# sumansamui/CMOOP_Audio_Processing

Measured on AMD Instinct MI355X. Metric: candidate-net evals/hour (pop=40, GSC-v2), higher is better.
Workload: dtype f32

## Files before the change

cmoop_audio_processing_amd/csrc/api.hip:

```cpp
#include "../../include/cmoop.h"
#include "net.h"

#include <cstring>
#include <mutex>
#include <vector>

using namespace cmoop;

static thread_local std::string g_err;
static thread_local std::string g_last_kernels;

template <class F>
static int guard(F&& f) {
    try {
        f();
        return 0;
    } catch (const std::exception& e) {
        g_err = e.what();
        return 1;
    } catch (...) {
        g_err = "unknown error";
        return 2;
    }
}
// ... 384 lines not shown
    return guard([&] {
        long long c = 0;
        h->net->read_train_metrics(loss_sum, &c, reset != 0);
        *correct = c;
    });
}
int cmoop_epoch_permutation(uint32_t seed, uint32_t epoch, int64_t n, int32_t* out_host) {
    return guard([&] { epoch_permutation(seed, epoch, n, out_host); });
}

int cmoop_epoch_permutation_device(uint32_t seed, uint32_t epoch, int64_t n, int32_t* out_dev) {
    return guard([&] {
        hipStream_t s = lib_stream();
        launch_epoch_permutation(seed, epoch, n, out_dev, s);
        CMOOP_HIP(hipStreamSynchronize(s));
    });
}


int cmoop_conv_fwd(const float* x, const float* w, const float* bias, float* y, int32_t B, int32_t H, int32_t W, int32_t Cin,
                   int32_t Cout, int32_t KS, int32_t stride, int32_t relu) {
    return guard([&] {
        g_last_kernels.clear();
        hipStream_t s = lib_stream();
        if (Cin == 1) {
            CMOOP_REQUIRE(stride == 1 && bias, "first-layer conv: stride 1 with bias");
            launch_conv1_fwd(x, nullptr, 0, w, bias, y, B, H, W, Cout, KS, relu, s);
        } else {
            GemmEpilogue e;
            e.bias = bias; e.relu = relu;
            const ConvGeom g = make_geom(B, H, W, Cin, Cout, KS, stride);
            const size_t skf = igemm_splitk_workspace(g);
            float* sk = nullptr;
            if (skf) CMOOP_HIP(hipMalloc(&sk, skf * 4));
            int flags = 0;
            const int code = launch_igemm_fwd(x, w, y, g, e, s, nullptr, sk, skf, nullptr, nullptr, 0, &flags);
            g_last_kernels = gemm_variant_name(0, code, flags);
            CMOOP_HIP(hipStreamSynchronize(s));
            if (sk) hipFree(sk);
        }
        CMOOP_HIP(hipStreamSynchronize(s));
    });
}

int cmoop_conv_bwd(const float* x, const float* w, const float* dy, float* dx, float* dw, float* db, int32_t B, int32_t H,
                   int32_t W, int32_t Cin, int32_t Cout, int32_t KS, int32_t stride, int32_t mask_relu) {
    return guard([&] {
        hipStream_t s = lib_stream();
        if (Cin == 1) {
            const int nb = conv1_wgrad_blocks(B, H, W);
            const int64_t per = (int64_t)Cout * (KS * KS + 1);
            float *P = nullptr, *tmp = nullptr;
            CMOOP_HIP(hipMalloc(&P, (size_t)nb * per * 4));
            CMOOP_HIP(hipMalloc(&tmp, (size_t)per * 4));
            launch_conv1_wgrad(x, nullptr, 0, dy, P, B, H, W, Cout, KS, s);
            launch_reduce_slices(P, tmp, nb, per, s);
            CMOOP_HIP(hipMemcpyAsync(dw, tmp, (size_t)Cout * KS * KS * 4, hipMemcpyDeviceToDevice, s));
            CMOOP_HIP(hipMemcpyAsync(db, tmp + (size_t)Cout * KS * KS, (size_t)Cout * 4, hipMemcpyDeviceToDevice, s));
            CMOOP_HIP(hipStreamSynchronize(s));
            hipFree(P); hipFree(tmp);
            return;
        }
        const ConvGeom g = make_geom(B, H, W, Cin, Cout, KS, stride);
        float *wg = nullptr, *red = nullptr, *wd = nullptr, *sk = nullptr;
        const size_t wg_floats = (size_t)wgrad_slices(g) * g.Cout * (g.K() + 1);
        CMOOP_HIP(hipMalloc(&wg, wg_floats * 4));
        CMOOP_HIP(hipMalloc(&red, ((size_t)1024 * 2 * Cout + 2 * Cout + 64) * 4));
        CMOOP_HIP(hipMalloc(&wd, (size_t)g.Cout * g.K() * 4));
        void* tab = nullptr;
        const int tab_rows = (KS * KS <= 32) ? rowtab_rows(g) : 0;
        if (tab_rows) {
            CMOOP_HIP(hipMalloc(&tab, (size_t)tab_rows * 8));
            launch_build_rowtab(g, tab, s);
        }
        g_last_kernels.clear();
        RecordingHook hook(&g_last_kernels);
        conv_backward_weights(x, dy, dw, db, g, wg, wg_floats, s, &hook, GEMM_DEFAULT, tab, tab_rows);
        if (dx) {
            int accumulate = 0;
            if (stride != 1) {
                CMOOP_HIP(hipMemsetAsync(dx, 0, (size_t)B * H * W * Cin * 4, s));
                accumulate = 1;
            }
            ConvGeom gd = g;
            gd.H = g.OH; gd.W = g.OW; gd.Cin = g.Cout; gd.Cout = g.Cin; gd.OH = g.H; gd.OW = g.W;
            const size_t skf = (stride == 1 && Cout >= 16 && (Cout & (Cout - 1)) == 0) ? igemm_splitk_workspace(gd) : 0;
            if (skf) CMOOP_HIP(hipMalloc(&sk, skf * 4));
            conv_backward_data(dy, w, dx, g, wd, mask_relu ? x : nullptr, 1.f, accumulate, s, &hook, sk, skf);
        }
        CMOOP_HIP(hipStreamSynchronize(s));
        hipFree(wg); hipFree(red); hipFree(wd);
        if (sk) hipFree(sk);
        if (tab) hipFree(tab);
    });
}

int cmoop_conv_fwd_trainer(const float* x, const float* w, const float* bias, float* y, int32_t B, int32_t H, int32_t W,
                           int32_t Cin, int32_t Cout, int32_t KS, int32_t stride, int32_t relu, double* col_sum,
                           double* col_sumsq, int32_t* stats_fused) {
    return guard([&] {
        g_last_kernels.clear();
        hipStream_t s = lib_stream();
        const ConvGeom g = make_geom(B, H, W, Cin, Cout, KS, stride);
        const int64_t M = g.M();
        GemmEpilogue e;
        e.bias = bias; e.relu = relu;
        float *sk = nullptr, *red = nullptr;
        void* tab = nullptr;
        const size_t skf = igemm_splitk_workspace(g);
        const bool want_stats = col_sum != nullptr && col_sumsq != nullptr;
        CMOOP_REQUIRE(!want_stats || Cout % 4 == 0, "statistics need Cout % 4 == 0");
        auto cleanup = [&] { hipStreamSynchronize(s); if (sk) hipFree(sk); if (red) hipFree(red); if (tab) hipFree(tab); };
        try {
            if (skf) CMOOP_HIP(hipMalloc(&sk, skf * 4));
            const int tab_rows = (KS * KS <= 32) ? rowtab_rows(g) : 0;
            if (tab_rows) {
                CMOOP_HIP(hipMalloc(&tab, (size_t)tab_rows * 8));
                launch_build_rowtab(g, tab, s);
            }
            size_t red_floats = 0;
            if (want_stats) {
                const size_t blocks = std::max<size_t>((size_t)colreduce_blocks(M, Cout), (size_t)cdiv64(M, 64));
                red_floats = blocks * 2 * Cout + 2 * Cout;
                CMOOP_HIP(hipMalloc(&red, red_floats * 4));
                e.stats = red;
            }
            int nb = 0, flags = 0;
            const int code = launch_igemm_fwd(x, w, y, g, e, s, nullptr, sk, skf, want_stats ? &nb : nullptr, tab, tab_rows, &flags);
            g_last_kernels = gemm_variant_name(0, code, flags);
            if (want_stats) {
                if (stats_fused) *stats_fused = nb > 0 ? 1 : 0;
                if (nb == 0) {
                    nb = colreduce_blocks(M, Cout);
                    launch_colstats(y, red, M, Cout, nb, s);
                }
                std::vector<float> hp((size_t)nb * 2 * Cout);
                CMOOP_HIP(hipMemcpyAsync(hp.data(), red, hp.size() * 4, hipMemcpyDeviceToHost, s));
                CMOOP_HIP(hipStreamSynchronize(s));
                for (int c = 0; c < Cout; ++c) { col_sum[c] = 0.0; col_sumsq[c] = 0.0; }
                for (int b = 0; b < nb; ++b)
                    for (int c = 0; c < Cout; ++c) {
                        col_sum[c] += (double)hp[((size_t)b * 2) * Cout + c];
                        col_sumsq[c] += (double)hp[((size_t)b * 2 + 1) * Cout + c];
                    }
            }
            CMOOP_HIP(hipStreamSynchronize(s));
        } catch (...) {
// ... 19 lines not shown
        try {
            RecordingHook hook(&g_last_kernels);
            const size_t NK = (size_t)g.Cout * g.K();
            const size_t wg_floats = (size_t)wgrad_slices(g) * g.Cout * (g.K() + 1);
            CMOOP_HIP(hipMalloc(&wg, wg_floats * 4));
            CMOOP_HIP(hipMalloc(&dwb, (NK + g.Cout) * 4));
            const int tab_rows = (KS * KS <= 32) ? rowtab_rows(g) : 0;
            if (tab_rows) {
                CMOOP_HIP(hipMalloc(&tab, (size_t)tab_rows * 8));
                launch_build_rowtab(g, tab, s);
            }
            conv_backward_weights(x, dy, dwb, dwb + NK, g, wg, wg_floats, s, &hook, GEMM_DEFAULT, tab, tab_rows);
            CMOOP_HIP(hipMemcpyAsync(dw, dwb, NK * 4, hipMemcpyDeviceToDevice, s));
            CMOOP_HIP(hipMemcpyAsync(db, dwb + NK, (size_t)g.Cout * 4, hipMemcpyDeviceToDevice, s));
            if (dx) {
                int accumulate = 0;
                if (stride != 1) {
                    CMOOP_HIP(hipMemsetAsync(dx, 0, (size_t)B * H * W * Cin * 4, s));
                    accumulate = 1;
                }
                const bool mfma_dgrad = ilog2_exact(Cout) >= 4;
                const ConvGeom gd = dgrad_geometry(g);
                int tab_d_rows = 0;
                size_t skf = 0;
                if (mfma_dgrad) {
                    CMOOP_HIP(hipMalloc(&wd, NK * 4));
                    launch_flip_transpose(w, wd, Cout, KS, KS, Cin, s);
                    if (KS * KS <= 32) {
                        tab_d_rows = rowtab_rows(gd);
                        CMOOP_HIP(hipMalloc(&tab_d, (size_t)tab_d_rows * 8));
                        launch_build_rowtab(gd, tab_d, s);
                    }
                    skf = igemm_splitk_workspace(gd);
                    if (skf) CMOOP_HIP(hipMalloc(&sk, skf * 4));
                }
                conv_backward_data(dy, w, dx, g, wd, mask_relu ? x : nullptr, 1.f, accumulate, s, &hook, sk, skf, GEMM_DEFAULT, mfma_dgrad,
                                   tab_d, tab_d_rows);
            }
            CMOOP_HIP(hipStreamSynchronize(s));
        } catch (...) {
            cleanup();
            throw;
        }
        cleanup();
    });
}

int cmoop_last_kernels(char* buf, int32_t cap) {
    return guard([&] {
        CMOOP_REQUIRE(buf && cap > 0, "last_kernels: no buffer");
        std::snprintf(buf, cap, "%s", g_last_kernels.c_str());
    });
}

int cmoop_conv_time(int32_t mode, const float* x, const float* w, const float* bias, float* y, int32_t B, int32_t H,
                    int32_t W, int32_t Cin, int32_t Cout, int32_t KS, int32_t iters, double* avg_ms) {
    return guard([&] {
        hipStream_t s = lib_stream();
        const ConvGeom g = make_geom(B, H, W, Cin, Cout, KS, 1);
        float *wd = nullptr, *wg = nullptr, *sk = nullptr;
        ConvGeom gd = g;
        GemmEpilogue e;
        const int S = wgrad_slices(g);
        if (mode == 0) e.bias = bias;
        if (mode == 1) {
            CMOOP_HIP(hipMalloc(&wd, (size_t)g.Cout * g.K() * 4));
            launch_flip_transpose(w, wd, Cout, KS, KS, Cin, s);
            gd.H = g.OH; gd.W = g.OW; gd.Cin = Cout; gd.Cout = Cin; gd.OH = g.H; gd.OW = g.W;
            gd.pad_t = KS - 1 - g.pad_t; gd.pad_l = KS - 1 - g.pad_l;
        }
        void* tab = nullptr;
        const int tab_rows = (KS * KS <= 32 && Cin >= 16) ? rowtab_rows(mode == 1 ? gd : g) : 0;
        if (mode == 2) CMOOP_HIP(hipMalloc(&wg, (size_t)S * g.Cout * g.K() * 4));
        if (tab_rows) {
            CMOOP_HIP(hipMalloc(&tab, (size_t)tab_rows * 8));
            launch_build_rowtab(mode == 1 ? gd : g, tab, s);
        }
        const size_t skf = mode == 0 ? igemm_splitk_workspace(g) : (mode == 1 ? igemm_splitk_workspace(gd) : 0);
        if (skf) CMOOP_HIP(hipMalloc(&sk, skf * 4));
        auto once = [&]() {
            if (mode == 0) launch_igemm_fwd(x, w, y, g, e, s, nullptr, sk, skf, nullptr, tab, tab_rows);
            else if (mode == 1) launch_igemm_fwd(y, wd, const_cast<float*>(x), gd, e, s, nullptr, sk, skf, nullptr, tab, tab_rows);
            else launch_igemm_wgrad(x, y, wg, g, S, s, nullptr, nullptr, 0, GEMM_DEFAULT, tab, tab_rows);
        };
        for (int i = 0; i < 3; ++i) once();
        hipEvent_t a, b;
        CMOOP_HIP(hipEventCreate(&a));
        CMOOP_HIP(hipEventCreate(&b));
        CMOOP_HIP(hipEventRecord(a, s));
        for (int i = 0; i < iters; ++i) once();
        CMOOP_HIP(hipEventRecord(b, s));
        CMOOP_HIP(hipEventSynchronize(b));
        float ms = 0.f;
        CMOOP_HIP(hipEventElapsedTime(&ms, a, b));
        hipEventDestroy(a); hipEventDestroy(b);
        if (wd) hipFree(wd);
        if (wg) hipFree(wg);
        if (sk) hipFree(sk);
        if (tab) hipFree(tab);
        *avg_ms = (double)ms / std::max(1, iters);
    });
}

int cmoop_dense_fwd(const float* x, const float* w, const float* bias, float* y, int32_t M, int32_t N, int32_t K, int32_t relu) {
    return guard([&] {
        hipStream_t s = lib_stream();
        launch_dense_fwd(x, w, bias, y, M, N, K, relu, 0, 0u, 0u, 1.f, GEMM_DEFAULT, s);
        CMOOP_HIP(hipStreamSynchronize(s));
    });
}
int cmoop_dense_bwd(const float* x, const float* w, const float* dy, float* dx, float* dw, float* db, int32_t M, int32_t N, int32_t K,
                    int32_t mask_relu) {
// ... 26 lines not shown
```

cmoop_audio_processing_amd/csrc/gemm.hip:

```cpp
#include "kernels.h"
#include <hip/hip_ext.h>
#include <cstdlib>
#include <mutex>
#include <string>
#include <type_traits>

namespace cmoop {

typedef float f32x4 __attribute__((ext_vector_type(4)));

typedef __bf16 bf16x8 __attribute__((ext_vector_type(8)));
typedef unsigned u32x4 __attribute__((ext_vector_type(4)));

typedef __bf16 bf16x2 __attribute__((ext_vector_type(2)));
typedef float f32x2 __attribute__((ext_vector_type(2)));

template <int NP>
__device__ __forceinline__ void split_pair(const float x, const float y, unsigned (&w)[NP]) {
    if constexpr (NP == 1) {
        w[0] = __builtin_bit_cast(unsigned, __builtin_convertvector((f32x2){x, y}, bf16x2));
    } else {
        const unsigned ux = __float_as_uint(x), uy = __float_as_uint(y);
        w[0] = __builtin_amdgcn_perm(uy, ux, 0x07060302u);
        const float rx = x - __uint_as_float(ux & 0xFFFF0000u), ry = y - __uint_as_float(uy & 0xFFFF0000u);
        const unsigned vx = __float_as_uint(rx), vy = __float_as_uint(ry);
        w[1] = __builtin_amdgcn_perm(vy, vx, 0x07060302u);
        const float sx = rx - __uint_as_float(vx & 0xFFFF0000u), sy = ry - __uint_as_float(vy & 0xFFFF0000u);
        w[2] = __builtin_amdgcn_perm(__float_as_uint(sy), __float_as_uint(sx), 0x07060302u);
    }
}

__device__ constexpr int X3_TA[6] = {2, 1, 0, 1, 0, 0};
__device__ constexpr int X3_TB[6] = {0, 1, 2, 0, 1, 0};

int gemm_mode_default() {
    static const int v = [] {
        const char* e = std::getenv("CMOOP_GEMM_MODE");
        if (!e) return (int)GEMM_FP32;
        const std::string m(e);
        return m == "bf16x3" ? (int)GEMM_BF16X3 : (m == "bf16" ? (int)GEMM_BF16 : (int)GEMM_FP32);
    }();
    return v;
}
static int resolve_mode(int mode) {
    const int m = mode >= 0 ? mode : gemm_mode_default();
    return (m == GEMM_BF16X3 || m == GEMM_BF16) ? m : GEMM_FP32;
}

struct GeomDev {
    int B, H, W, Cin, OH, OW, Cout, KH, KW, stride, pad_t, pad_l;
    int M, K, cshift, OHW;
    uint32_t ohw_magic, ohw_shift, ow_magic, ow_shift;
    int rcp_kw;
    const float* zeros;
};
struct EpiDev {
    int bal_L, bal_segmax;
    float* stats;
    const float* bias;
    const float* mask;
    float mask_scale;
    int relu, accumulate, out_stride, OHf, OWf, dropout;
    uint32_t drop_prefix, drop_thr;
    float drop_scale;
};

static double par_scale() {
    static const double v = [] {
        const char* e = std::getenv("CMOOP_PAR_SCALE");
        const double x = e ? std::atof(e) : 1.0;
        return x > 0.01 && x <= 4.0 ? x : 1.0;
    }();
    return v;
}

static void fastdiv_init(int d, uint32_t* magic, uint32_t* shift) {
    uint32_t s = 0;
    while ((1u << s) < (uint32_t)d) ++s;
    *shift = s;
    *magic = (uint32_t)((((uint64_t)1 << 32) * (((uint64_t)1 << s) - (uint64_t)d)) / (uint64_t)d + 1);
}
__device__ __forceinline__ int fastdiv(int n, uint32_t magic, uint32_t shift) {
    return (int)((__umulhi((uint32_t)n, magic) + (uint32_t)n) >> shift);
}

static const float* zero_page() {
    static thread_local const float* page[16] = {nullptr};
    int dev = 0;
    CMOOP_HIP(hipGetDevice(&dev));
    CMOOP_REQUIRE(dev >= 0 && dev < 16, "device index out of range");
// ... 569 lines not shown
                const int c = wcol + ct * 16 + lr;
                red[((wave / WN) * BN + c) * 2] = csum[ct];
                red[((wave / WN) * BN + c) * 2 + 1] = csq[ct];
            }
        }
        __syncthreads();
        if (t < BN && n0 + t < N) {
            float a = 0.f, b = 0.f;
#pragma unroll
            for (int w = 0; w < WM; ++w) { a += red[(w * BN + t) * 2]; b += red[(w * BN + t) * 2 + 1]; }
            e.stats[((size_t)mtile * 2) * N + n0 + t] = a;
            e.stats[((size_t)mtile * 2 + 1) * N + n0 + t] = b;
        }
    }
    }
}

struct HaloDev {
    int WP, rows_max, VH;
    uint32_t wp_magic, wp_shift, vh_magic, vh_shift;
};
__host__ __device__ constexpr int halo_nst(int bm) { return bm == 256 ? 11 : 9; }
static bool halo_geometry(const ConvGeom& cg, HaloDev* hd, size_t* lds_bytes);
static size_t halo_balanced_slab_floats(const ConvGeom& cg, int* L_out);

template <int KS, int BM, int BN, int WM, bool BAL = false>
__global__ __launch_bounds__(256, 2) void halo_fwd_kernel(const float* __restrict__ X, const float* __restrict__ Wt,
                                                          float* __restrict__ Y, GeomDev g, EpiDev e, HaloDev h,
                                                          float* __restrict__ slab) {
    constexpr int WN = 4 / WM, RT = BM / WM / 16, CT = BN / WN / 16, R = KS / 2, T = KS * KS;
    constexpr int PITCH = 24;
    constexpr int NST = halo_nst(BM);
    static_assert(RT >= 1 && CT >= 1, "tile too small for the wave layout");
    extern __shared__ __attribute__((aligned(16))) float halo[];

    const int t = threadIdx.x;
    const int ncc = g.Cin >> 4;
    const int upt = ncc * KS;
    int u = 0, uend = 1;
    if constexpr (BAL) {
        const int U = ((g.M + BM - 1) / BM) * ((g.Cout + BN - 1) / BN) * upt;
        u = blockIdx.x * e.bal_L;
        uend = min(U, u + e.bal_L);
    }
    while (u < uend) {
    int mtile, ntile, c_lo = 0, c_hi = upt;
    float* pslab = nullptr;
    if constexpr (BAL) {
        const int nt = (g.Cout + BN - 1) / BN;
        const int t0 = u / upt;
        c_lo = u - t0 * upt;
        c_hi = min(upt, c_lo + (uend - u));
        mtile = t0 / nt; ntile = t0 - mtile * nt;
        const int seg = c_lo == 0 ? 0 : (int)blockIdx.x - (t0 * upt) / e.bal_L;
        pslab = slab + ((size_t)t0 * e.bal_segmax + seg) * (BM * BN);
        u += c_hi - c_lo;
        __syncthreads();
    } else {
        u = uend;
        mtile = blockIdx.x;
        const int nwg = gridDim.x, xcd = mtile & 7, idx = mtile >> 3;
        const int qn = nwg >> 3, rn = nwg & 7;
        mtile = (xcd < rn ? xcd * (qn + 1) : rn * (qn + 1) + (xcd - rn) * qn) + idx;
        ntile = blockIdx.y;
    }
    const int m0 = mtile * BM, n0 = ntile * BN;
    const int wave = t >> 6, lane = t & 63, lr = lane & 15, q = lane >> 4;
    const int wrow = (wave / WN) * (BM / WM), wcol = (wave % WN) * (BN / WN);

    auto vrow = [&](int m, int& x) {
        const int b = fastdiv(m, g.ohw_magic, g.ohw_shift), r = m - b * g.OHW;
        const int y = fastdiv(r, g.ow_magic, g.ow_shift);
        x = r - y * g.OW;
        return b * h.VH + y;
    };
    int xdummy;
    const int vbase = vrow(m0, xdummy);
    const int vlast = vrow(min(m0 + BM, g.M) - 1, xdummy);
    const int items = (vlast - vbase + 1 + 2 * R) * h.WP * 4;

    const __amdgpu_buffer_rsrc_t xr = __builtin_amdgcn_make_buffer_rsrc(
        const_cast<float*>(X), 0, (int)((uint32_t)g.B * g.H * g.W << g.cshift) * 4, 0x00020000);
    const __amdgpu_buffer_rsrc_t wr = __builtin_amdgcn_make_buffer_rsrc(const_cast<float*>(Wt), 0, g.Cout * g.K * 4, 0x00020000);
    uint32_t s_voff[NST];
#pragma unroll
    for (int it = 0; it < NST; ++it) {
        const int i = t + 256 * it, pix = i >> 2, j = i & 3;
// ... 67 lines not shown
                    for (int rt = 0; rt < RT; ++rt)
                        an[rt] = *reinterpret_cast<const f32x4*>(a_ptr[rt] + ky * wp_f + (kx + 1) * PITCH);
                } else if (!last_unit) {
                    load_b(ncc2, nky * KS, bn);
                    if (!new_cc) {
#pragma unroll
                        for (int rt = 0; rt < RT; ++rt) an[rt] = *reinterpret_cast<const f32x4*>(a_ptr[rt] + nky * wp_f);
                    }
                }
                __builtin_amdgcn_s_setprio(1);
#pragma unroll
                for (int j = 0; j < 4; ++j)
#pragma unroll
                    for (int rt = 0; rt < RT; ++rt)
#pragma unroll
                        for (int ct = 0; ct < CT; ++ct)
                            acc[rt][ct] = __builtin_amdgcn_mfma_f32_16x16x4f32(ac[rt][j], bc[ct][j], acc[rt][ct], 0, 0, 0);
                __builtin_amdgcn_s_setprio(0);
#pragma unroll
                for (int ct = 0; ct < CT; ++ct) bc[ct] = bn[ct];
                if (kx + 1 < KS || (!last_unit && !new_cc)) {
#pragma unroll
                    for (int rt = 0; rt < RT; ++rt) ac[rt] = an[rt];
                } else if (!last_unit) {
                    __syncthreads();
                    stage_store();
                    __syncthreads();
#pragma unroll
                    for (int rt = 0; rt < RT; ++rt) ac[rt] = *reinterpret_cast<const f32x4*>(a_ptr[rt]);
                }
            }
            ky = nky; cc = ncc2;
        }
#pragma unroll
        for (int rt = 0; rt < RT; ++rt)
#pragma unroll
            for (int r = 0; r < 4; ++r)
#pragma unroll
                for (int ct = 0; ct < CT; ++ct)
                    pslab[(wrow + rt * 16 + q * 4 + r) * BN + wcol + ct * 16 + lr] = acc[rt][ct][r];
        continue;
    } else {
    f32x4 ac[RT], bc[CT];
    stage_load(0);
    load_b(0, 0, bc);
    stage_store();
    __syncthreads();
#pragma unroll
    for (int rt = 0; rt < RT; ++rt) ac[rt] = *reinterpret_cast<const f32x4*>(a_ptr[rt]);

    for (int cc = 0; cc < ncc; ++cc) {
        const bool more = cc + 1 < ncc;
#pragma unroll
        for (int tap = 0; tap < T; ++tap) {
            f32x4 an[RT], bn[CT];
#pragma unroll
            for (int ct = 0; ct < CT; ++ct) bn[ct] = bc[ct];
            if (tap + 1 < T) {
                load_b(cc, tap + 1, bn);
                const int ky = (tap + 1) / KS, kx = (tap + 1) % KS;
#pragma unroll
                for (int rt = 0; rt < RT; ++rt)
                    an[rt] = *reinterpret_cast<const f32x4*>(a_ptr[rt] + ky * wp_f + kx * PITCH);
            } else if (more) {
                load_b(cc + 1, 0, bn);
            }
            if (tap == T - 2 && more) stage_load(cc + 1);
            __builtin_amdgcn_s_setprio(1);
#pragma unroll
            for (int j = 0; j < 4; ++j)
#pragma unroll
                for (int rt = 0; rt < RT; ++rt)
#pragma unroll
                    for (int ct = 0; ct < CT; ++ct)
// ... 68 lines not shown
                    float v = (mk[r][ct] > 0.f) ? acc[rt][ct][r] * e.mask_scale : 0.f;
                    if (e.accumulate) v += old[r][ct];
                    __builtin_amdgcn_raw_buffer_store_b32(__float_as_uint(v), yrs, (int)(e_lane + ct * 64), soff, 0);
                }
        }
    } else {
#pragma unroll
    for (int rt = 0; rt < RT; ++rt) {
#pragma unroll
        for (int r = 0; r < 4; ++r) {
            const int row = m0 + wrow + rt * 16 + q * 4 + r;
            if (row >= g.M) continue;
            const size_t rbase = (size_t)row * N;
#pragma unroll
            for (int ct = 0; ct < CT; ++ct) {
                const int col = n0 + wcol + ct * 16 + lr;
                if (col >= N) continue;
                float v = acc[rt][ct][r] + bias_v[ct];
                if (e.relu) v = fmaxf(v, 0.f);
                const size_t off = rbase + col;
                if (e.dropout) {
                    uint32_t u24 = fmix32(e.drop_prefix ^ (uint32_t)((size_t)row * N + col)) >> 8;
                    v = (u24 >= e.drop_thr) ? v * e.drop_scale : 0.f;
                }
                if (e.mask) v = (e.mask[off] > 0.f) ? v * e.mask_scale : 0.f;
                if (e.accumulate) v += Y[off];
                Y[off] = v;
                csum[ct] += v;
                csq[ct] += v * v;
            }
        }
    }
    }
    if (e.stats) {
        __syncthreads();
        float* red = halo;
#pragma unroll
        for (int ct = 0; ct < CT; ++ct) {
            csum[ct] += __shfl_xor(csum[ct], 16, 64);
            csq[ct] += __shfl_xor(csq[ct], 16, 64);
            csum[ct] += __shfl_xor(csum[ct], 32, 64);
            csq[ct] += __shfl_xor(csq[ct], 32, 64);
            if (q == 0) {
                const int c = wcol + ct * 16 + lr;
                red[((wave / WN) * BN + c) * 2] = csum[ct];
                red[((wave / WN) * BN + c) * 2 + 1] = csq[ct];
            }
        }
        __syncthreads();
        if (t < BN && n0 + t < N) {
            float a = 0.f, b = 0.f;
#pragma unroll
            for (int w = 0; w < WM; ++w) { a += red[(w * BN + t) * 2]; b += red[(w * BN + t) * 2 + 1]; }
            e.stats[((size_t)mtile * 2) * N + n0 + t] = a;
            e.stats[((size_t)mtile * 2 + 1) * N + n0 + t] = b;
        }
    }
    }
}

struct BalDev { int bm, bn, nt, chunks, L, segmax; };

template <int VEC>
__global__ __launch_bounds__(256) void splitk_combine_kernel(const float* __restrict__ P, float* __restrict__ Y, GeomDev g,
                                                             EpiDev e, int splits, BalDev bal) {
    const int N = g.Cout;
    const size_t total = (size_t)g.M * N;
// ... 136 lines not shown
    if (balanced_on) {
        int W = 0;
        const size_t need = balanced_slab_floats(M, N, K, bk, bn_big, &W);
        if (need > 0 && need <= ws_floats) { *bm = 128; *bn = bn_big; *balanced_wgs = W; return; }
    }
    if (nchunks >= (M <= 512 ? 4 : 16) && ws_floats > 0) {
        const int min_chunks = M <= 512 ? 2 : 8;
        int sp = (int)std::min<long>(cdiv((int)(1024 * par_scale()), (int)blocks), nchunks / min_chunks);
        sp = std::min(sp, 32);
        if (sp > 1) sp = fill_waves(blocks, sp, std::max(32, (int)(512 * par_scale())));
        while (sp > 1 && (size_t)sp * M * N > ws_floats) --sp;
        if (sp > 1) {
            const int cps = cdiv(nchunks, sp);
            sp = cdiv(nchunks, cps);
            *bm = 128; *bn = bn_big; *splits = sp;
            return;
        }
    }
    blocks = (long)cdiv(M, 128) * cdiv(N, bn_small);
    if (blocks >= fill) { *bm = 128; *bn = bn_small; return; }
    *bm = 64; *bn = bn_small;
}

size_t igemm_splitk_workspace(const ConvGeom& g) {
    const int M = g.M(), N = g.Cout;
    const int bn_big = N > 64 ? 128 : (N <= 16 ? 16 : (N <= 32 ? 32 : 64));
    const long blocks = (long)cdiv(M, 128) * cdiv(N, bn_big);
    if (blocks >= 384) return 0;
    const int sp = std::min(32, cdiv(1024, (int)blocks));
    return std::max(std::max((size_t)sp * M * N, balanced_slab_floats(M, N, g.K(), g.Cin % 32 == 0 ? 32 : 16, bn_big, nullptr)),
                    halo_balanced_slab_floats(g, nullptr));
}

static size_t halo_balanced_slab_floats(const ConvGeom& cg, int* L_out) {
    static const bool on = [] { const char* v = std::getenv("CMOOP_HALO_BAL"); return !(v && v[0] == '0'); }();
    if (!on || cg.Cout % 64 != 0 || !halo_geometry(cg, nullptr, nullptr)) return 0;
    const long tiles = (long)cdiv(cg.M(), 128) * (cg.Cout / 64);
    const int upt = (cg.Cin / 16) * cg.KH;
    const long units = tiles * upt;
    if (tiles >= 1024 || units < 512l * 2 * cg.KH) return 0;
    const int L = (int)((units + 511) / 512);
    if (L_out) *L_out = L;
    return (size_t)tiles * (cdiv(upt, L) + 1) * 128 * 64;
}

struct FwdChoice {
    int mode, bm, bn, splits, balanced_wgs, flags;
    bool bk32_tile, use_dma, stats, halo;
    int ks, halo_L;
    int code() const { return mode * 100000000 + bm * 100000 + bn * 100 + (halo ? ks + (halo_L > 0 ? 50 : 0) : (bk32_tile ? 32 : 16)); }
};

static inline int halo_bm(int cout) { return cout >= 64 ? 128 : 256; }
static bool halo_geometry(const ConvGeom& cg, HaloDev* hd, size_t* lds_bytes) {
    const int ks = cg.KH, R = ks / 2;
    if (cg.KH != cg.KW || (ks != 3 && ks != 5) || cg.stride != 1 || cg.OH != cg.H || cg.OW != cg.W) return false;
    if (cg.pad_t != R || cg.pad_l != R || cg.Cin % 16 != 0) return false;
    if (cg.Cout % 64 != 0 && cg.Cout != 32 && cg.Cout != 16) return false;
    const int bm = halo_bm(cg.Cout);
    const int wp = (cg.W + ks - 1 + 7) / 8 * 8;
    const int span = (bm - 2 + cg.W) / cg.W + 1 + ((bm - 1) / (cg.H * cg.W) + 1) * R;
    const int rows = span + 2 * R;
    if (rows * wp * 4 > halo_nst(bm) * 256) return false;
    const size_t lds = (size_t)rows * wp * 24 * sizeof(float);
    if (lds > 64 * 1024) return false;
    if (hd) {
        hd->WP = wp; hd->rows_max = rows; hd->VH = cg.H + R;
        fastdiv_init(wp, &hd->wp_magic, &hd->wp_shift);
        fastdiv_init(cg.H + R, &hd->vh_magic, &hd->vh_shift);
    }
    if (lds_bytes) *lds_bytes = lds;
    return true;
}
// ... 41 lines not shown
        }
    }
    c.flags = (c.splits > 1 ? GEMM_FLAG_SPLITK : 0) | (c.stats ? GEMM_FLAG_STATS : 0) | (c.balanced_wgs ? GEMM_FLAG_BALANCED : 0) |
              ((!c.halo && have_rowtab && (cg.Cin % bk) == 0 && cg.KH * cg.KW <= 32) ? GEMM_FLAG_ROWTAB : 0);
    return c;
}

int igemm_fwd_plan(const ConvGeom& g, const GemmEpilogue& ep, size_t ws_floats, bool want_stats, bool have_rowtab, int* flags_out) {
    igemm_check_range(g);
    CMOOP_REQUIRE(ilog2_exact(g.Cin) >= 4, "implicit GEMM needs C_in a power of two >= 16");
    const FwdChoice c = choose_fwd(g, ep, ws_floats, want_stats, have_rowtab);
    if (flags_out) *flags_out = c.flags;
    return c.code();
}

int launch_igemm_fwd(const float* X, const float* Wt, float* Y, const ConvGeom& cg, const GemmEpilogue& ep,
                     hipStream_t s, const GemmTiming* tm, float* splitk_ws, size_t splitk_ws_floats, int* stats_blocks,
                     const void* rowtab_v, int tab_rows, int* flags_out) {
    if (stats_blocks) *stats_blocks = 0;
    if (flags_out) *flags_out = 0;
    const uint2* rowtab = static_cast<const uint2*>(rowtab_v);
    GeomDev g = to_dev(cg);
    if (g.M == 0) return 0;
    EpiDev e;
    e.bias = ep.bias; e.mask = ep.mask; e.mask_scale = ep.mask_scale; e.relu = ep.relu;
    e.accumulate = ep.accumulate; e.out_stride = ep.out_stride; e.OHf = ep.OHf; e.OWf = ep.OWf;
    e.dropout = ep.dropout; e.drop_prefix = ep.drop_prefix; e.drop_thr = ep.drop_thr; e.drop_scale = ep.drop_scale;
    if (e.out_stride > 1)
        CMOOP_REQUIRE((int64_t)g.B * e.OHf * e.OWf * g.Cout < (1ll << 29), "scattered output too large");
    const FwdChoice ch = choose_fwd(cg, ep, splitk_ws ? splitk_ws_floats : 0, ep.stats != nullptr && stats_blocks != nullptr, rowtab != nullptr);
    const int mode = ch.mode == GEMM_FP32_DMA ? (int)GEMM_FP32 : ch.mode;
    const int bm = ch.bm, bn = ch.bn, splits = ch.splits, balanced_wgs = ch.balanced_wgs;
    const bool bk32_tile = ch.bk32_tile, use_dma = ch.use_dma;
    e.bal_L = 0; e.bal_segmax = 0;
    e.stats = ch.stats ? ep.stats : nullptr;
    if (e.stats) *stats_blocks = cdiv(g.M, bm);
    if (flags_out) *flags_out = ch.flags;
    if (ch.halo) {
        HaloDev hd;
        size_t lds = 0;
        CMOOP_REQUIRE(halo_geometry(cg, &hd, &lds), "halo kernel chosen for a geometry it does not accept");
        dim3 grid(cdiv(g.M, bm), cdiv(g.Cout, bn));
        BalDev bal{bm, bn, cdiv(g.Cout, bn), (cg.Cin / 16) * cg.KH, ch.halo_L, 0};
        if (ch.halo_L > 0) {
            bal.segmax = cdiv(bal.chunks, bal.L) + 1;
            e.bal_L = bal.L; e.bal_segmax = bal.segmax;
            const long units = (long)grid.x * grid.y * bal.chunks;
            grid = dim3((unsigned)((units + bal.L - 1) / bal.L), 1, 1);
            lds = std::max(lds, (size_t)55 * 1024);
        }
        {
            static const int occ_env = [] { const char* v = std::getenv("CMOOP_HALO_OCC"); return v ? std::atoi(v) : 0; }();
            const long wgs = (long)grid.x * grid.y;
            auto fill = [&](long slots) { return (double)wgs / (double)(((wgs + slots - 1) / slots) * slots); };
            const bool two = occ_env == 2 || (occ_env != 3 && lds <= 53 * 1024 && wgs <= 1536 && fill(512) > fill(768) + 0.05);
            if (two) lds = std::max(lds, (size_t)55 * 1024);
        }
#define CMOOP_HALO_LAUNCH(KS_, BM_, BN_, WM_, BAL_)                                                                                        \
        do {                                                                                                                 \
            if (tm && tm->start && tm->ext) {                                                                                \
                hipExtLaunchKernelGGL((halo_fwd_kernel<KS_, BM_, BN_, WM_, BAL_>), grid, dim3(256), lds, s, tm->start, tm->stop, 0, X, Wt, Y, g, e, hd, splitk_ws); \
            } else {                                                                                                         \
                if (tm && tm->start) CMOOP_HIP(hipEventRecord(tm->start, s));                                                \
                hipLaunchKernelGGL((halo_fwd_kernel<KS_, BM_, BN_, WM_, BAL_>), grid, dim3(256), lds, s, X, Wt, Y, g, e, hd, splitk_ws);    \
                if (tm && tm->start) CMOOP_HIP(hipEventRecord(tm->stop, s));                                                 \
            }                                                                                                                \
        } while (0)
#define CMOOP_HALO_KS(KS_)                                                                     \
        do {                                                                                   \
            if (ch.halo_L > 0) CMOOP_HALO_LAUNCH(KS_, 128, 64, 2, true);                       \
            else if (bn == 64) CMOOP_HALO_LAUNCH(KS_, 128, 64, 2, false);                      \
            else if (bn == 32) CMOOP_HALO_LAUNCH(KS_, 256, 32, 4, false);                      \
            else CMOOP_HALO_LAUNCH(KS_, 256, 16, 4, false);                                    \
        } while (0)
        if (cg.KH == 5) CMOOP_HALO_KS(5); else CMOOP_HALO_KS(3);
#undef CMOOP_HALO_KS
#undef CMOOP_HALO_LAUNCH
        CMOOP_HIP(hipGetLastError());
        if (ch.halo_L > 0) {
            const size_t total = (size_t)g.M * g.Cout;
            const unsigned gridc = (unsigned)std::min<size_t>((total / 4 + 255) / 256, 4096);
            hipLaunchKernelGGL(splitk_combine_kernel<4>, dim3(gridc), dim3(256), 0, s, splitk_ws, Y, g, e, 2, bal);
            CMOOP_HIP(hipGetLastError());
        }
        return ch.code();
    }
#define CMOOP_FWD(BM_, BN_, WM_)                                                              \
    do {                                                                                      \
        if (mode == GEMM_BF16X3) launch_fwd_t<BM_, BN_, 32, WM_, GEMM_BF16X3>(X, Wt, Y, g, e, s, tm, splitk_ws, splits, balanced_wgs, rowtab, tab_rows);   \
        else if (mode == GEMM_BF16) launch_fwd_t<BM_, BN_, 32, WM_, GEMM_BF16>(X, Wt, Y, g, e, s, tm, splitk_ws, splits, balanced_wgs, rowtab, tab_rows);  \
        else if (use_dma && BM_ == 128 && BN_ == 32) launch_fwd_t<BM_, 32, 32, WM_, GEMM_FP32_DMA>(X, Wt, Y, g, e, s, tm, splitk_ws, splits, balanced_wgs, rowtab, tab_rows);   \
        else if (bk32_tile) launch_fwd_t<BM_, BN_, 32, WM_>(X, Wt, Y, g, e, s, tm, splitk_ws, splits, balanced_wgs, rowtab, tab_rows);   \
        else launch_fwd_t<BM_, BN_, 16, WM_>(X, Wt, Y, g, e, s, tm, splitk_ws, splits, 0, rowtab, tab_rows);        \
    } while (0)
    if (bm == 128) {
        if (bn == 128) CMOOP_FWD(128, 128, 2);
        else if (bn == 64) CMOOP_FWD(128, 64, 4);
        else if (bn == 32) CMOOP_FWD(128, 32, 4);
        else CMOOP_FWD(128, 16, 4);
    } else {
        if (bn == 64) CMOOP_FWD(64, 64, 2);
        else if (bn == 32) CMOOP_FWD(64, 32, 4);
        else CMOOP_FWD(64, 16, 4);
    }
#undef CMOOP_FWD
    return ch.code();
}

__global__ __launch_bounds__(256) void build_rowtab_kernel(GeomDev g, uint2* __restrict__ tab, int rows_padded) {
    const int m = blockIdx.x * 256 + threadIdx.x;
    if (m >= rows_padded) return;
    if (m >= g.M) { tab[m] = make_uint2(0u, 0xFFFFFFFFu); return; }
// ... 826 lines not shown
```

cmoop_audio_processing_amd/csrc/kernels.h:

```cpp
#pragma once
#include "common.h"
#include <string>

namespace cmoop {

struct ConvGeom {
    int B, H, W, Cin;
    int OH, OW, Cout;
    int KH, KW, stride;
    int pad_t, pad_l;
    int M() const { return B * OH * OW; }
    int K() const { return KH * KW * Cin; }
};

enum GemmMode { GEMM_DEFAULT = -1, GEMM_FP32 = 0, GEMM_FP32_DMA = 1 , GEMM_BF16X3 = 2, GEMM_BF16 = 3,
                GEMM_FP32_HALO = 4  };
int gemm_mode_default();

struct GemmEpilogue {
    int mode = GEMM_DEFAULT;
    const float* bias = nullptr;
    int relu = 0;
    const float* mask = nullptr;
    float mask_scale = 1.f;
    int accumulate = 0;
    int out_stride = 1;
    int OHf = 0, OWf = 0;
    int dropout = 0;
    uint32_t drop_prefix = 0, drop_thr = 0;
    float drop_scale = 1.f;
    float* stats = nullptr;
};

struct GemmTiming {
    hipEvent_t start = nullptr, stop = nullptr;
    bool ext = true;
};
enum GemmFlags { GEMM_FLAG_SPLITK = 1, GEMM_FLAG_STATS = 2, GEMM_FLAG_ROWTAB = 4, GEMM_FLAG_BALANCED = 8, GEMM_FLAG_SLABS = 16 };
int launch_igemm_fwd(const float* X, const float* Wt, float* Y, const ConvGeom& g,
                     const GemmEpilogue& e, hipStream_t s, const GemmTiming* tm = nullptr,
                     float* splitk_ws = nullptr, size_t splitk_ws_floats = 0, int* stats_blocks = nullptr,
                     const void* rowtab = nullptr, int tab_rows = 0, int* flags_out = nullptr);
size_t igemm_splitk_workspace(const ConvGeom& g);
int igemm_fwd_plan(const ConvGeom& g, const GemmEpilogue& e, size_t ws_floats, bool want_stats, bool have_rowtab, int* flags_out);
int igemm_wgrad_plan(const ConvGeom& g, int S, int mode, bool have_rowtab, int* flags_out);
void halo_rows_bound_and_need(const ConvGeom& g, int* bound, int* need, int* items_cap);
void igemm_check_range(const ConvGeom& g);
std::string gemm_kernel_name(int cls, int code);

int wgrad_slices(const ConvGeom& g);
int launch_igemm_wgrad(const float* X, const float* dY, float* P, const ConvGeom& g, int S, hipStream_t s,
                       const GemmTiming* tm = nullptr, float* Pbias = nullptr, size_t slab_stride = 0,
                       int mode = GEMM_DEFAULT, const void* rowtab = nullptr, int tab_rows = 0, int* flags_out = nullptr);
int rowtab_rows(const ConvGeom& g);
void launch_build_rowtab(const ConvGeom& g, void* tab, hipStream_t s);
void launch_reduce_slices(const float* P, float* out, int S, int64_t n, hipStream_t s, int64_t stride = 0);
void launch_flip_transpose(const float* W, float* Wd, int Cout, int KH, int KW, int Cin, hipStream_t s);
struct FlipEntry { int64_t w_off, wd_off; int Cout, KH, KW, Cin; };
void launch_flip_transpose_all(const float* params, float* wd_all, const FlipEntry* table_dev, int layers, int64_t max_elems,
                               hipStream_t s);

struct StepState {
    long long row0;
    unsigned step;
    unsigned iter;
};
void launch_step_advance(StepState* st, int batch, hipStream_t s);
void launch_glorot_init(float* w, int64_t n, uint32_t prefix, float scale, hipStream_t s);
void launch_fill(float* w, float v, int64_t n, hipStream_t s);

void launch_dense_fwd(const float* X, const float* W, const float* bias, float* Y, int M, int N, int K, int relu,
                      int dropout, uint32_t drop_prefix, uint32_t drop_thr, float drop_scale, int mode, hipStream_t s,
                      const StepState* st = nullptr, uint32_t drop_seed = 0, uint32_t drop_stream = 0);
void launch_dense_dgrad(const float* dY, const float* W, float* dX, int M, int N, int K, const float* mask, float mask_scale,
                        int mode, hipStream_t s);
void launch_dense_wgrad(const float* X, const float* dY, float* dW, float* dB, int M, int N, int K, int mode, hipStream_t s);
// ... 80 lines not shown
```

cmoop_audio_processing_amd/csrc/net.hip:

```cpp
#include "net.h"

#include <algorithm>
#include <chrono>
#include <cmath>
#include <cstdlib>
#include <cstring>
#include <functional>
#include <map>
#include <numeric>
#include <thread>

namespace cmoop {

static const int FC_LADDER[5][4] = {{0, 0, 0, 0}, {64, 0, 0, 0}, {128, 64, 0, 0}, {256, 128, 64, 0}, {512, 256, 128, 64}};

void validate_gene(const int32_t g[6]) {
    const bool ok = (g[0] == 16 || g[0] == 32 || g[0] == 64) && (g[1] == 3 || g[1] == 5) && (g[2] == 0 || g[2] == 1) &&
                    (g[3] >= 1 && g[3] <= 3) && (g[4] >= 1 && g[4] <= 4) && (g[5] == 0 || g[5] == 1);
    CMOOP_REQUIRE(ok, "gene outside the search space (filters{16,32,64}, kernel{3,5}, bn{0,1}, res{1..3}, fc{1..4}, dropout{0,1})");
}

int64_t param_count(const int32_t g[6], int variant, int classes) {
    validate_gene(g);
    const int64_t f = g[0], kk = (int64_t)g[1] * g[1], bn = g[2], R = g[3], fc = g[4];
// ... 335 lines not shown
            const int64_t M = g.M();
            if (op.Cout % 4 == 0)
                red_ws_floats_ = std::max(red_ws_floats_, (size_t)colreduce_blocks(M, op.Cout) * 2 * op.Cout + 2 * op.Cout);
        }
        if (op.kind == OP_CONV1) {
            const size_t per = (size_t)op.Cout * (op.KS * op.KS + 1);
            for (int b = 1; b <= cfg_.batch; ++b) op.slab_floats = std::max(op.slab_floats, per * conv1_wgrad_blocks(b, T_, F_));
            op.slab_off = (int64_t)wgrad_ws_floats_;
            wgrad_ws_floats_ += (op.slab_floats + 3) / 4 * 4;
            red_ws_floats_ = std::max(red_ws_floats_, (size_t)colreduce_blocks((int64_t)Bmax_ * T_ * F_, op.Cout) * 2 * op.Cout + 2 * op.Cout);
        }
        if (op.kind == OP_BN) {
            const int64_t M = (int64_t)Bmax_ * acts_[op.in].H * acts_[op.in].W;
            const size_t blocks = std::max<size_t>((size_t)colreduce_blocks(M, op.Cout), (size_t)cdiv64(M, 64));
            red_ws_floats_ = std::max(red_ws_floats_, blocks * 2 * op.Cout + 2 * op.Cout);
        }
    }
    wgrad_ws_ = dalloc(wgrad_ws_floats_);
    wd_ws_ = dalloc(wd_ws_floats_);
    {
        std::vector<FlipEntry> tab;
        for (const auto& op : ops_)
            if (op.kind == OP_CONV && op.wd_off >= 0) {
                tab.push_back(FlipEntry{op.w_off, op.wd_off, op.Cout, op.KS, op.KS, op.Cin});
                flip_max_elems_ = std::max<int64_t>(flip_max_elems_, (int64_t)op.Cout * op.KS * op.KS * op.Cin);
            }
        flip_layers_ = (int)tab.size();
        if (flip_layers_) {
            flip_table_ = reinterpret_cast<FlipEntry*>(dalloc(tab.size() * sizeof(FlipEntry) / sizeof(float) + 4));
            CMOOP_HIP(hipMemcpyAsync(flip_table_, tab.data(), tab.size() * sizeof(FlipEntry), hipMemcpyHostToDevice, stream_));
            CMOOP_HIP(hipStreamSynchronize(stream_));
        }
    }
    splitk_ws_ = splitk_ws_floats_ ? dalloc(splitk_ws_floats_) : nullptr;
    red_ws_ = dalloc(red_ws_floats_ + 64);
    acc_train_ = reinterpret_cast<double*>(dalloc(8));
    acc_eval_ = acc_train_ + 2;
    CMOOP_HIP(hipMemsetAsync(acc_train_, 0, 32, stream_));
    if (cfg_.profile_every > 0) {
        ev_pool_.resize(1024);
        const char* pm = std::getenv("CMOOP_PROFILE_PAIRS");
        const bool ext = !(pm && pm[0] == '1');
        static std::atomic<bool> said{false};
        if (!said.exchange(true)) std::fprintf(stderr, "[cmoop] GEMM launch timing: %s\n", ext ? "hipExtLaunchKernelGGL events" : "hipEventRecord pairs");
        for (auto& e : ev_pool_) {
            CMOOP_HIP(hipEventCreate(&e.t.start));
            CMOOP_HIP(hipEventCreate(&e.t.stop));
            e.t.ext = ext;
        }
    }
}

ConvGeom Net::geom_of(const Op& op, int B) const {
    const Act& ia = acts_[op.in];
    ConvGeom g;
    g.B = B; g.H = ia.H; g.W = ia.W; g.Cin = op.Cin;
    g.OH = (ia.H + op.stride - 1) / op.stride; g.OW = (ia.W + op.stride - 1) / op.stride; g.Cout = op.Cout;
    g.KH = g.KW = op.KS; g.stride = op.stride;
    const int th = std::max((g.OH - 1) * op.stride + op.KS - ia.H, 0);
    const int tw = std::max((g.OW - 1) * op.stride + op.KS - ia.W, 0);
    g.pad_t = th / 2; g.pad_l = tw / 2;
    return g;
}

void Net::get_params(float* host) {
    CMOOP_HIP(hipMemcpyAsync(host, params_, n_params_ * 4, hipMemcpyDeviceToHost, stream_));
    CMOOP_HIP(hipStreamSynchronize(stream_));
// ... 684 lines not shown
```

Measured before the change: 441.0.

## Fuse balanced halo split-K reduction into GEMM via per-tile atomic fix-up

Replaces the separate split-K combine kernel for the balanced halo GEMM with an in-kernel fix-up. Each segment stores its partial tile to the slab and bumps a per-tile atomic counter, and the last-arriving workgroup sums all partials and runs the normal epilogue. This removes one kernel launch and a full slab read/write pass over the output. In exchange it needs counter storage appended to the split-K workspace, a zeroing memset at allocation, and correct memory ordering. Fused stats are disabled on this path.

Result: no change. 443.8, median of 6 (+0.6%).

```diff
diff --git a/cmoop_audio_processing_amd/csrc/api.hip b/cmoop_audio_processing_amd/csrc/api.hip
--- a/cmoop_audio_processing_amd/csrc/api.hip
+++ b/cmoop_audio_processing_amd/csrc/api.hip
@@ -440,7 +440,10 @@
             const ConvGeom g = make_geom(B, H, W, Cin, Cout, KS, stride);
             const size_t skf = igemm_splitk_workspace(g);
             float* sk = nullptr;
-            if (skf) CMOOP_HIP(hipMalloc(&sk, skf * 4));
+            if (skf) {
+                CMOOP_HIP(hipMalloc(&sk, igemm_splitk_alloc_floats(skf) * 4));
+                igemm_splitk_zero_counters(sk, skf, s);
+            }
             int flags = 0;
             const int code = launch_igemm_fwd(x, w, y, g, e, s, nullptr, sk, skf, nullptr, nullptr, 0, &flags);
             g_last_kernels = gemm_variant_name(0, code, flags);
@@ -493,7 +496,10 @@
             ConvGeom gd = g;
             gd.H = g.OH; gd.W = g.OW; gd.Cin = g.Cout; gd.Cout = g.Cin; gd.OH = g.H; gd.OW = g.W;
             const size_t skf = (stride == 1 && Cout >= 16 && (Cout & (Cout - 1)) == 0) ? igemm_splitk_workspace(gd) : 0;
-            if (skf) CMOOP_HIP(hipMalloc(&sk, skf * 4));
+            if (skf) {
+                CMOOP_HIP(hipMalloc(&sk, igemm_splitk_alloc_floats(skf) * 4));
+                igemm_splitk_zero_counters(sk, skf, s);
+            }
             conv_backward_data(dy, w, dx, g, wd, mask_relu ? x : nullptr, 1.f, accumulate, s, &hook, sk, skf);
         }
         CMOOP_HIP(hipStreamSynchronize(s));
@@ -520,7 +526,10 @@
         CMOOP_REQUIRE(!want_stats || Cout % 4 == 0, "statistics need Cout % 4 == 0");
         auto cleanup = [&] { hipStreamSynchronize(s); if (sk) hipFree(sk); if (red) hipFree(red); if (tab) hipFree(tab); };
         try {
-            if (skf) CMOOP_HIP(hipMalloc(&sk, skf * 4));
+            if (skf) {
+                CMOOP_HIP(hipMalloc(&sk, igemm_splitk_alloc_floats(skf) * 4));
+                igemm_splitk_zero_counters(sk, skf, s);
+            }
             const int tab_rows = (KS * KS <= 32) ? rowtab_rows(g) : 0;
             if (tab_rows) {
                 CMOOP_HIP(hipMalloc(&tab, (size_t)tab_rows * 8));
@@ -606,7 +615,10 @@
                         launch_build_rowtab(gd, tab_d, s);
                     }
                     skf = igemm_splitk_workspace(gd);
-                    if (skf) CMOOP_HIP(hipMalloc(&sk, skf * 4));
+                    if (skf) {
+                        CMOOP_HIP(hipMalloc(&sk, igemm_splitk_alloc_floats(skf) * 4));
+                        igemm_splitk_zero_counters(sk, skf, s);
+                    }
                 }
                 conv_backward_data(dy, w, dx, g, wd, mask_relu ? x : nullptr, 1.f, accumulate, s, &hook, sk, skf, GEMM_DEFAULT, mfma_dgrad,
                                    tab_d, tab_d_rows);
@@ -651,7 +663,10 @@
             launch_build_rowtab(mode == 1 ? gd : g, tab, s);
         }
         const size_t skf = mode == 0 ? igemm_splitk_workspace(g) : (mode == 1 ? igemm_splitk_workspace(gd) : 0);
-        if (skf) CMOOP_HIP(hipMalloc(&sk, skf * 4));
+        if (skf) {
+            CMOOP_HIP(hipMalloc(&sk, igemm_splitk_alloc_floats(skf) * 4));
+            igemm_splitk_zero_counters(sk, skf, s);
+        }
         auto once = [&]() {
             if (mode == 0) launch_igemm_fwd(x, w, y, g, e, s, nullptr, sk, skf, nullptr, tab, tab_rows);
             else if (mode == 1) launch_igemm_fwd(y, wd, const_cast<float*>(x), gd, e, s, nullptr, sk, skf, nullptr, tab, tab_rows);
diff --git a/cmoop_audio_processing_amd/csrc/gemm.hip b/cmoop_audio_processing_amd/csrc/gemm.hip
--- a/cmoop_audio_processing_amd/csrc/gemm.hip
+++ b/cmoop_audio_processing_amd/csrc/gemm.hip
@@ -56,6 +56,7 @@
 };
 struct EpiDev {
     int bal_L, bal_segmax;
+    int* bal_cnt;
     float* stats;
     const float* bias;
     const float* mask;
@@ -691,6 +692,7 @@
     constexpr int PITCH = 24;
     constexpr int NST = halo_nst(BM);
     static_assert(RT >= 1 && CT >= 1, "tile too small for the wave layout");
+    static_assert(!BAL || RT * CT * 1024 == BM * BN, "fix-up slab slot: one 16-byte store per accumulator and thread");
     extern __shared__ __attribute__((aligned(16))) float halo[];
 
     const int t = threadIdx.x;
@@ -704,6 +706,7 @@
     }
     while (u < uend) {
     int mtile, ntile, c_lo = 0, c_hi = upt;
+    int tile = 0, seg = 0, nseg = 1;
     float* pslab = nullptr;
     if constexpr (BAL) {
         const int nt = (g.Cout + BN - 1) / BN;
@@ -711,7 +714,10 @@
         c_lo = u - t0 * upt;
         c_hi = min(upt, c_lo + (uend - u));
         mtile = t0 / nt; ntile = t0 - mtile * nt;
-        const int seg = c_lo == 0 ? 0 : (int)blockIdx.x - (t0 * upt) / e.bal_L;
+        const int first = (t0 * upt) / e.bal_L;
+        tile = t0;
+        seg = c_lo == 0 ? 0 : (int)blockIdx.x - first;
+        nseg = ((t0 + 1) * upt + e.bal_L - 1) / e.bal_L - first;
         pslab = slab + ((size_t)t0 * e.bal_segmax + seg) * (BM * BN);
         u += c_hi - c_lo;
         __syncthreads();
@@ -845,14 +851,62 @@
             }
             ky = nky; cc = ncc2;
         }
+        if (!e.bal_cnt) {
+#pragma unroll
+            for (int rt = 0; rt < RT; ++rt)
+#pragma unroll
+                for (int r = 0; r < 4; ++r)
+#pragma unroll
+                    for (int ct = 0; ct < CT; ++ct)
+                        pslab[(wrow + rt * 16 + q * 4 + r) * BN + wcol + ct * 16 + lr] = acc[rt][ct][r];
+            continue;
+        }
+        const __amdgpu_buffer_rsrc_t srs = __builtin_amdgcn_make_buffer_rsrc(slab + (size_t)tile * e.bal_segmax * (BM * BN), 0,
+                                                                             e.bal_segmax * (BM * BN) * 4, 0x00020000);
+        if (nseg > 1) {
+#pragma unroll
+            for (int rt = 0; rt < RT; ++rt)
+#pragma unroll
+                for (int ct = 0; ct < CT; ++ct)
+                    __builtin_amdgcn_raw_buffer_store_b128(__builtin_bit_cast(u32x4, acc[rt][ct]), srs, t * 16,
+                                                           ((seg * RT + rt) * CT + ct) * 4096, 16);
+            asm volatile("s_waitcnt vmcnt(0)" ::: "memory");
+            __syncthreads();
+            int* const bcast = reinterpret_cast<int*>(halo);
+            if (t == 0) {
+                const int old = __hip_atomic_fetch_add(e.bal_cnt + tile, 1, __ATOMIC_RELAXED, __HIP_MEMORY_SCOPE_AGENT);
+                if (old == nseg - 1) {
+                    __hip_atomic_store(e.bal_cnt + tile, 0, __ATOMIC_RELAXED, __HIP_MEMORY_SCOPE_AGENT);
+                    __builtin_amdgcn_fence(__ATOMIC_ACQUIRE, "agent");
+                    asm volatile("s_waitcnt vmcnt(0)" ::: "memory");
+                }
+                *bcast = old;
+            }
+            __syncthreads();
+            if (__builtin_amdgcn_readfirstlane(*bcast) != nseg - 1) continue;
+        }
+        f32x4 sum[RT][CT];
 #pragma unroll
         for (int rt = 0; rt < RT; ++rt)
 #pragma unroll
-            for (int r = 0; r < 4; ++r)
+            for (int ct = 0; ct < CT; ++ct) sum[rt][ct] = f32x4{0.f, 0.f, 0.f, 0.f};
+        for (int z = 0; z < nseg; ++z) {
+            f32x4 p[RT][CT];
+#pragma unroll
+            for (int rt = 0; rt < RT; ++rt)
 #pragma unroll
                 for (int ct = 0; ct < CT; ++ct)
-                    pslab[(wrow + rt * 16 + q * 4 + r) * BN + wcol + ct * 16 + lr] = acc[rt][ct][r];
-        continue;
+                    p[rt][ct] = z == seg ? acc[rt][ct]
+                                         : __builtin_bit_cast(f32x4, __builtin_amdgcn_raw_buffer_load_b128(srs, t * 16, ((z * RT + rt) * CT + ct) * 4096, 0));
+#pragma unroll
+            for (int rt = 0; rt < RT; ++rt)
+#pragma unroll
+                for (int ct = 0; ct < CT; ++ct) sum[rt][ct] += p[rt][ct];
+        }
+#pragma unroll
+        for (int rt = 0; rt < RT; ++rt)
+#pragma unroll
+            for (int ct = 0; ct < CT; ++ct) acc[rt][ct] = sum[rt][ct];
     } else {
     f32x4 ac[RT], bc[CT];
     stage_load(0);
@@ -987,7 +1041,7 @@
         }
     }
     }
-    if (e.stats) {
+    if (!BAL && e.stats) {
         __syncthreads();
         float* red = halo;
 #pragma unroll
@@ -1190,13 +1244,17 @@
                     halo_balanced_slab_floats(g, nullptr));
 }
 
+void igemm_splitk_zero_counters(float* splitk_ws, size_t slab_floats, hipStream_t s) {
+    if (splitk_ws && slab_floats) CMOOP_HIP(hipMemsetAsync(splitk_ws + slab_floats, 0, IGEMM_TILE_COUNTERS * sizeof(int), s));
+}
+
 static size_t halo_balanced_slab_floats(const ConvGeom& cg, int* L_out) {
     static const bool on = [] { const char* v = std::getenv("CMOOP_HALO_BAL"); return !(v && v[0] == '0'); }();
     if (!on || cg.Cout % 64 != 0 || !halo_geometry(cg, nullptr, nullptr)) return 0;
     const long tiles = (long)cdiv(cg.M(), 128) * (cg.Cout / 64);
     const int upt = (cg.Cin / 16) * cg.KH;
     const long units = tiles * upt;
-    if (tiles >= 1024 || units < 512l * 2 * cg.KH) return 0;
+    if (tiles >= (long)IGEMM_TILE_COUNTERS || units < 512l * 2 * cg.KH) return 0;
     const int L = (int)((units + 511) / 512);
     if (L_out) *L_out = L;
     return (size_t)tiles * (cdiv(upt, L) + 1) * 128 * 64;
@@ -1304,7 +1362,7 @@
     const int mode = ch.mode == GEMM_FP32_DMA ? (int)GEMM_FP32 : ch.mode;
     const int bm = ch.bm, bn = ch.bn, splits = ch.splits, balanced_wgs = ch.balanced_wgs;
     const bool bk32_tile = ch.bk32_tile, use_dma = ch.use_dma;
-    e.bal_L = 0; e.bal_segmax = 0;
+    e.bal_L = 0; e.bal_segmax = 0; e.bal_cnt = nullptr;
     e.stats = ch.stats ? ep.stats : nullptr;
     if (e.stats) *stats_blocks = cdiv(g.M, bm);
     if (flags_out) *flags_out = ch.flags;
@@ -1317,6 +1375,8 @@
         if (ch.halo_L > 0) {
             bal.segmax = cdiv(bal.chunks, bal.L) + 1;
             e.bal_L = bal.L; e.bal_segmax = bal.segmax;
+            const char* fx = std::getenv("CMOOP_HALO_FIXUP");
+            if (!(fx && fx[0] == '0')) e.bal_cnt = reinterpret_cast<int*>(splitk_ws + splitk_ws_floats);
             const long units = (long)grid.x * grid.y * bal.chunks;
             grid = dim3((unsigned)((units + bal.L - 1) / bal.L), 1, 1);
             lds = std::max(lds, (size_t)55 * 1024);
@@ -1349,7 +1409,7 @@
 #undef CMOOP_HALO_KS
 #undef CMOOP_HALO_LAUNCH
         CMOOP_HIP(hipGetLastError());
-        if (ch.halo_L > 0) {
+        if (ch.halo_L > 0 && !e.bal_cnt) {
             const size_t total = (size_t)g.M * g.Cout;
             const unsigned gridc = (unsigned)std::min<size_t>((total / 4 + 255) / 256, 4096);
             hipLaunchKernelGGL(splitk_combine_kernel<4>, dim3(gridc), dim3(256), 0, s, splitk_ws, Y, g, e, 2, bal);
diff --git a/cmoop_audio_processing_amd/csrc/kernels.h b/cmoop_audio_processing_amd/csrc/kernels.h
--- a/cmoop_audio_processing_amd/csrc/kernels.h
+++ b/cmoop_audio_processing_amd/csrc/kernels.h
@@ -42,6 +42,9 @@
                      float* splitk_ws = nullptr, size_t splitk_ws_floats = 0, int* stats_blocks = nullptr,
                      const void* rowtab = nullptr, int tab_rows = 0, int* flags_out = nullptr);
 size_t igemm_splitk_workspace(const ConvGeom& g);
+constexpr size_t IGEMM_TILE_COUNTERS = 1024;
+inline size_t igemm_splitk_alloc_floats(size_t slab_floats) { return slab_floats ? slab_floats + IGEMM_TILE_COUNTERS : 0; }
+void igemm_splitk_zero_counters(float* splitk_ws, size_t slab_floats, hipStream_t s);
 int igemm_fwd_plan(const ConvGeom& g, const GemmEpilogue& e, size_t ws_floats, bool want_stats, bool have_rowtab, int* flags_out);
 int igemm_wgrad_plan(const ConvGeom& g, int S, int mode, bool have_rowtab, int* flags_out);
 void halo_rows_bound_and_need(const ConvGeom& g, int* bound, int* need, int* items_cap);
diff --git a/cmoop_audio_processing_amd/csrc/net.hip b/cmoop_audio_processing_amd/csrc/net.hip
--- a/cmoop_audio_processing_amd/csrc/net.hip
+++ b/cmoop_audio_processing_amd/csrc/net.hip
@@ -391,7 +391,8 @@
             CMOOP_HIP(hipStreamSynchronize(stream_));
         }
     }
-    splitk_ws_ = splitk_ws_floats_ ? dalloc(splitk_ws_floats_) : nullptr;
+    splitk_ws_ = splitk_ws_floats_ ? dalloc(igemm_splitk_alloc_floats(splitk_ws_floats_)) : nullptr;
+    igemm_splitk_zero_counters(splitk_ws_, splitk_ws_floats_, stream_);
     red_ws_ = dalloc(red_ws_floats_ + 64);
     acc_train_ = reinterpret_cast<double*>(dalloc(8));
     acc_eval_ = acc_train_ + 2;
```
